# 123456jack/decision-making-and-path-planning

Measured on AMD Instinct MI355X. Metric: planning ticks/sec (batched scenes), 512x512 grid, higher is better.
Workload: dtype f64; 1 GPU; BASELINE configs[1]: 1024 scenes/GPU, 512x512 grid, 64 static obstacles; scenes_per_gpu=1024, global_scenes=1024, grid=512, obstacles=64, parallelism=scene-sharded x1, RCCL scatter/gather outside the timed region, algorithmic_bytes_per_tick=276644

## Files before the change

### decision-making-and-path-planning_amd/__init__.py

```python
import ctypes as C
import os

import numpy as np

_HERE = os.path.dirname(os.path.abspath(__file__))
LIB_PATH = os.path.join(_HERE, "libdmpp.so")

PATH_POINTS, OUT_POINTS, LANESUM, MAX_REFPATH, MAX_LATTICE = 200, 100, 8, 512, 17
GEN_LANE_PTS, GEN_REF_PTS = 320, 128

G_FOUND, G_NO_PATH, G_LIMIT, G_OVERFLOW, G_GOAL_BLOCKED, G_PATH_TRUNC, G_INTERNAL, G_COST_RANGE = range(8)
G_STATUS_COUNT = 8
K_NAMES = ["k_effective_obstacles", "k_decision", "k_planning", "k_search", "k_score"]
(BUF_SCENE_IN, BUF_LANE_POOL, BUF_REF_POOL, BUF_OBS_POOL, BUF_MOT_POOL, BUF_STATE, BUF_PLAN_OUT, BUF_GRID_OUT,
 BUF_GRID, BUF_PATH, BUF_ORDER, BUF_LANE_ATTR) = range(12)


def _dt(fields):
    return np.dtype(fields, align=True)


f8, i4, u4, f4, u8, u2 = np.float64, np.int32, np.uint32, np.float32, np.uint64, np.uint16
GlobalPoint2D = _dt([("x", f8), ("y", f8)])
GlobalPoint3D = _dt([("x", f8), ("y", f8), ("dir", f8)])
AimPoint = _dt([("Aim_point", GlobalPoint3D), ("Aim_id", i4), ("_pad", i4)])
ObPoint = _dt([("x", f8), ("y", f8), ("type", i4), ("radius", f4)])
ObMotion = _dt([("vx", f8), ("vy", f8)])
LaneView = _dt([("cur_off", i4), ("cur_n", i4), ("left_off", i4), ("left_n", i4), ("right_off", i4), ("right_n", i4),
                ("lane_sum", i4), ("lanechg_attribute", i4), ("lane_width", f8)])
LocationOut = _dt([("globalpoint", GlobalPoint3D), ("velocity", f8), ("pos", i4), ("road_num", i4), ("lane_num", i4),
                   ("last_roadnum", i4), ("next_roadnum", i4), ("last_lanenum", i4), ("next_lanenum", i4),
                   ("path_num", i4), ("id", i4, (LANESUM,))])
DecisionOutPod = _dt([("velocity_expect", f8), ("behavior", i4), ("target_roadnum", i4), ("target_lanenum", i4),
                   ("light", i4), ("behavior_to_dlg", i4), ("refpath_n", i4)])
Obs_To_Veh = _dt([("dis_lat", f8), ("dis_lng", f8)])
Path_Obs = _dt([("Ob_Pose", Obs_To_Veh), ("Ob_Attr", ObPoint), ("Obs_flag", i4), ("Ob_Pathid", i4)])
PlanningOut = _dt([("brakedis", f8), ("brake_speed", f8), ("desacc", f8), ("desspd", f8), ("desstr", f8), ("radius", f8),
                   ("cnt", i4), ("APA", i4), ("desaccVd", i4), ("desstrVd", i4), ("light", i4), ("road_type", i4),
# ... 728 lines not shown
```

### decision-making-and-path-planning_amd/csrc/dmpp_hip.hip

```cpp
#include <hip/hip_runtime.h>
#include <cstddef>
#include <cstdio>
#include <cstring>
#include <cmath>
#include <string>
#include <cstdlib>
#include <vector>
#include <new>
#include <algorithm>
#include "../../include/dmpp_planner.h"
#include "kernels_r.hpp"
#include "kernels_a.hpp"
#include "kernels_rt.hpp"
#include "kernels_ep.hpp"
#include "kernels_es.hpp"
#include "kernels_g.hpp"
#include "kernels_sc.hpp"
#include "kernels_f.hpp"
#include "kernels_t.hpp"
#include "kernels_op.hpp"
#include "search_budget.hpp"

namespace {

// ... 150 lines not shown
    DevBuf<int32_t> d_perm[kBuf], d_cost[kBuf];
    DevBuf<uint2> d_ospill[kBuf]; int spill_cap = 0; DevBuf<int32_t> d_retry[kBuf];
    hipStream_t stream_m[kBuf] = {};
    size_t grid_cells = 0;
    int bucket_cap0 = 0, max_path0 = 0;
    int search_kind = 0; int search_meta_bytes = 0; int lds_budget = 0, lds_budget_max = 0; bool lds_budget_fixed = false, search_force_gbm = false, budget_from_need = false;
    int gbm_lds = 0; int search_slots = 512; size_t search_static_lds = 0;
    DevBuf<int32_t> d_ovf[kBuf], d_need[kObs]; HostPin<int32_t> h_need;
    int need_seen = 0;
    DevBuf<int> d_gridbad;
    int gcap = 1, tick_group = 0;
    int grp_ticks = 0, grp_G = 1, grp_n = 0, grp_p_prev = 0; bool grp_piped = false;
    int grp_set[kGroupMax] = {}, grp_gs[kGroupMax] = {}; const SceneIn* grp_in = nullptr;
    int ring = 0, gring = 0;
    int item_off = 0;
    int need_set = 0;

    hipStream_t stream_r = nullptr; SyncPoint fork, join;
    SyncPoint searched[kBuf], scored[kObs], raster;
    bool front_unjoined = false;
    int parity = 0;
    bool last_piped = false;
    int obs_set = 0;
    int n_cus = 256;
    int pipeline_min = 256;
    bool r_on_main = false;
    DevBuf<char> d_scratch;
    bool streaming = false;
    InputSet in_sets[kIn]; int in_cur = 0, in_staged = -1;
    DevBuf<PlanOut> d_plan_ring[kPlan]; int plan_cur = 0;
    hipStream_t stream_up = nullptr, stream_dp = nullptr, stream_dg = nullptr;
    SyncPoint fetched_plan[kPlan], fetched_grid[kGout];
    SyncPoint done_p[kDone], done_g[kDone]; long long done_tick[kDone];
    HostPin<int32_t> h_bad;
    long long tick_seq = 0;
    TickRec rec_last = { -1, 0, nullptr, nullptr };
    std::vector<TickRec> inflight; std::vector<hipEvent_t> sync_events;
    std::vector<PendingFetch> fetches;
    RolloutState rollout;
    ScoreState score;
    FleetState fleet;
    RouteState route;
    TrafficState traffic;
    FollowState follow;
    EpisodeState episode;
    SpawnState spawn;
// ... 316 lines not shown

}

extern "C" {

const char* pp_last_error(void) { return g_err.c_str(); }

int pp_create(const PlannerConfig* cfg, int device, const PlannerCaps* caps, pp_handle* out)
{
    if (!out || !caps) return fail(PP_ERR_ARG, "null argument");
    *out = nullptr;
    int r = check_cfg(cfg); if (r) return r;
    if (caps->max_scenes <= 0) return fail(PP_ERR_ARG, "max_scenes must be positive");
    int ndev = 0;
    hipError_t e = hipGetDeviceCount(&ndev);
    if (e != hipSuccess || ndev <= 0) return fail(PP_ERR_HIP, std::string("no HIP device: ") + hipGetErrorString(e));
    if (device < 0 || device >= ndev) return fail(PP_ERR_ARG, "device index out of range");
    HIP_TRY(hipSetDevice(device));
    pp_planner* h = new (std::nothrow) pp_planner();
    if (!h) return fail(PP_ERR_HIP, "out of host memory");
    h->cfg = *cfg; h->caps = *caps; h->device = device;
    if (const char* e = std::getenv("DMPP_PIPELINE_MIN")) h->pipeline_min = std::atoi(e);
    if (const char* e = std::getenv("DMPP_TICK_GROUP")) h->tick_group = std::atoi(e);
    if (cfg->grid_stage) {
        const size_t cells = (size_t)cfg->grid_w * cfg->grid_h;
        const size_t item_bytes = cells * sizeof(uint16_t) + 3 * (cells / 32) * sizeof(uint32_t) + (size_t)std::max(caps->order_cap, 0) * sizeof(int32_t) +
                                  (cfg->bucket_cap > DMPP_OPEN_CAP ? (size_t)cfg->bucket_cap * sizeof(uint2) : 0) + 4 * sizeof(int32_t);
        h->gcap = group_cap(caps->max_scenes, h->pipeline_min, h->tick_group, item_bytes);
    }
    auto bail = [&](int code) { pp_destroy(h); return code; };
    int prio_least = 0, prio_greatest = 0;
    (void)hipDeviceGetStreamPriorityRange(&prio_least, &prio_greatest);
    const int prio_normal = (prio_least + prio_greatest) / 2;
    if (hipStreamCreateWithPriority(&h->stream, hipStreamNonBlocking, prio_normal) != hipSuccess) return bail(fail(PP_ERR_HIP, "hipStreamCreate failed"));
    h->stream_m[0] = h->stream;
    for (int q = 1; q < kBuf; q++)
        if (hipStreamCreateWithPriority(&h->stream_m[q], hipStreamNonBlocking, prio_normal) != hipSuccess) return bail(fail(PP_ERR_HIP, "hipStreamCreate failed"));
    hipDeviceProp_t prop;
    if (hipGetDeviceProperties(&prop, device) == hipSuccess) h->n_cus = prop.multiProcessorCount;
    if (hipStreamCreateWithPriority(&h->stream_r, hipStreamNonBlocking, prio_greatest) != hipSuccess) return bail(fail(PP_ERR_HIP, "hipStreamCreate failed"));
    if ((r = h->fork.create()) || (r = h->join.create())) return bail(r);
    const size_t ns = (size_t)caps->max_scenes;
    if ((r = h->in_sets[0].d_in.reserve(ns))) return bail(r);
    if ((r = h->d_lane.reserve((size_t)caps->max_lane_pts_total))) return bail(r);
    if ((r = h->d_attr.reserve((size_t)caps->max_lane_pts_total + 1))) return bail(r);
    if ((r = h->d_ref.reserve((size_t)caps->max_ref_pts_total))) return bail(r);
// ... 394 lines not shown
    const int gs = c.grid_stage ? h->gring * kGroupMax + slot : h->gout_set;
    if (h->streaming) {
        int r = pump_fetches(h, -1, (h->plan_cur + 1) % kPlan, c.grid_stage ? gs : -1); if (r) return r;
        r = prune_inflight(h); if (r) return r;
        h->plan_cur = (h->plan_cur + 1) % kPlan; h->d_plan = h->d_plan_ring[h->plan_cur];
        if (!adopted) h->h_bad[(h->tick_seq + 1) % kDone] = 0;
    }
    const TickStreams T = tick_streams(h, piped, c.grid_stage != 0, h->parity);
    hipStream_t sf = T.front, sr = T.dp;
    PP_TRY(h->scored[po].wait(sf));
    if (sf == h->stream && h->front_unjoined) PP_TRY(h->join.wait(sf));
    h->front_unjoined = false;
    if (h->r_on_main && sf != h->stream) {
        PP_TRY(h->fork.record(h->stream)); PP_TRY(h->fork.wait(sf));
    }
    h->r_on_main = sr == h->stream;
    const SyncPoint& up = h->in_sets[h->in_cur].up;
    const bool behind_upload = adopted && up.recorded();
    if (behind_upload) PP_TRY(up.wait_unless_done(sf));
    if (h->streaming) PP_TRY(h->fetched_plan[h->plan_cur].wait_unless_done(sr));
    if (h->score.ego.done()) h->score.ego.forget();
    else if (!behind_upload) PP_TRY(h->score.ego.wait(sf));
    ObPoint* obs_now = h->d_obs_now[po];
    {
        Timed t(h, PP_K_OBSTACLES, sf);
        hipLaunchKernelGGL(dmpp::k_effective_obstacles, dim3(n), dim3(dmpp::kBlock), 0, sf, c, n, h->d_in, h->d_state,
                           h->d_obs, h->have_motion ? h->d_mot : nullptr, obs_now);
    }
    if (sr != sf) { PP_TRY(h->fork.record(sf)); PP_TRY(h->fork.wait(sr)); }
    if (c.grid_stage && sf != T.search) PP_TRY(h->raster.record(sf));
    if (c.decision_stage) {
        Timed t(h, PP_K_DECISION, sr);
        hipLaunchKernelGGL(dmpp::k_decision, dim3(n), dim3(dmpp::kBlock), sizeof(dmpp::DecShared), sr, c, n, h->d_in, h->d_lane,
                           h->d_attr, h->d_ref, obs_now, h->d_state, h->d_plan, h->d_dec_ref);
    }
    {
        Timed t(h, PP_K_PLANNING, sr);
        hipLaunchKernelGGL(dmpp::k_planning, dim3(n), dim3(dmpp::kBlock), sizeof(dmpp::PlanShared), sr, c, n, h->d_in, h->d_lane,
                           h->d_ref, h->d_dec_ref, obs_now, h->d_state, h->d_plan);
    }
    if (sr != h->stream) { PP_TRY(h->join.record(sr)); h->front_unjoined = piped; }
    h->obs_set = po;
    if (c.grid_stage) {
        h->grp_set[slot] = po; h->grp_gs[slot] = gs; h->grp_in = h->d_in;
        h->grp_ticks = slot + 1;
        h->gout_set = gs; h->path_set = po;
        h->score.grp_scored = h->score.on;
        if (slot + 1 == G) { int r = flush_group(h); if (r) return r; }
    }
    h->last_piped = piped;
    h->tick_seq++;
    if (h->streaming) {
        TickRec rec = { h->tick_seq, h->in_cur, get_sync_event(h), c.grid_stage ? get_sync_event(h) : nullptr };
        if (!rec.ev_front || (c.grid_stage && !rec.ev_tail)) return fail(PP_ERR_HIP, "event creation failed");
        HIP_TRY(hipEventRecord(rec.ev_front, sr));
        if (rec.ev_tail) HIP_TRY(hipEventRecord(rec.ev_tail, T.score));
        h->inflight.push_back(rec); h->rec_last = rec;
        if (h->score.on) {
// ... 1119 lines not shown
    if (!h) return fail(PP_ERR_ARG, "null handle");
    int r = drain_events(h); if (r) return r;
    for (int k = 0; k < PP_K_COUNT; k++) { h->k_ms[k] = 0; h->k_launches[k] = 0; }
    return PP_OK;
}
void* pp_device_ptr(pp_handle h, int which, size_t* bytes)
{
    if (!h) return nullptr;
    if (flush_group(h)) return nullptr;
    const size_t ns = (size_t)h->caps.max_scenes;
    void* p = nullptr; size_t b = 0;
    switch (which) {
    case PP_BUF_SCENE_IN: p = h->d_in; b = ns * sizeof(SceneIn); break;
    case PP_BUF_LANE_POOL: p = h->d_lane; b = (size_t)h->caps.max_lane_pts_total * sizeof(GlobalPoint3D); break;
    case PP_BUF_REF_POOL: p = h->d_ref; b = (size_t)h->caps.max_ref_pts_total * sizeof(GlobalPoint2D); break;
    case PP_BUF_OBS_POOL: p = h->d_obs; b = (size_t)h->caps.max_obs_total * sizeof(ObPoint); break;
    case PP_BUF_MOT_POOL: p = h->d_mot; b = (size_t)h->caps.max_obs_total * sizeof(ObMotion); break;
    case PP_BUF_STATE: p = h->d_state; b = ns * sizeof(SceneState); break;
    case PP_BUF_PLAN_OUT: p = h->d_plan; b = ns * sizeof(PlanOut); break;
    case PP_BUF_GRID_OUT: p = h->d_gout[h->gout_set]; b = ns * sizeof(GridOut); break;
    case PP_BUF_GRID: p = nullptr; b = 0; break;
    case PP_BUF_PATH: p = h->d_path[h->path_set]; b = ns * (size_t)h->max_path0 * 4; break;
    case PP_BUF_LANE_ATTR: p = h->d_attr; b = (size_t)h->caps.max_lane_pts_total; break;
    case PP_BUF_ORDER: p = h->d_order[h->parity] ? h->d_order[h->parity] + (size_t)h->item_off * h->caps.order_cap : nullptr; b = ns * (size_t)h->caps.order_cap * 4; break;
    default: break;
    }
    if (bytes) *bytes = b;
    return p;
}
int pp_tick_group_size(int n_scenes, int search_slots, int gcap, int forced) { return group_size(n_scenes, search_slots, gcap, forced); }
int pp_tick_group_cap(int max_scenes, int pipeline_min, int forced, size_t item_bytes) { return group_cap(max_scenes, pipeline_min, forced, item_bytes); }
int pp_tick_group_const(int which)
{
    switch (which) {
    case 0: return kGroupMax;
    case 1: return kBuf;
    case 2: return kRing;
    case 3: return kObs;
    case 4: return kGoutRing;
    case 5: return kGout;
    default: return -1;
    }
}
int pp_search_budget(int static_lds, int meta_bytes, int gbm_lds, int lds_budget_max, int n_cus, int n_scenes, int group, int n_obs_total,
                     int need, int budget, int from_need, int mode, int32_t* budget_out, int32_t* from_need_out, int32_t* slots_out)
{
// ... 29 lines not shown
```

### decision-making-and-path-planning_amd/csrc/kernels_r.hpp

```cpp
#pragma once
#include "dev_geom.hpp"

#ifndef DMPP_FRONT_PRIO
#define DMPP_FRONT_PRIO 3
#endif
namespace dmpp {

constexpr int kBlock = 256;

#ifdef DMPP_DEBUG_SEARCH
#define FRONT_MARK(slot) { if (threadIdx.x == 0) dbg_stamp[slot] = (double)(clock64() - dbg_t0); }
#else
#define FRONT_MARK(slot)
#endif
constexpr int kMaxObsLds = 512;

__global__ void __launch_bounds__(kBlock)
k_effective_obstacles(PlannerConfig c, int n_scenes, const SceneIn* __restrict__ in, const SceneState* __restrict__ st,
                      const ObPoint* __restrict__ obs, const ObMotion* __restrict__ mot, ObPoint* __restrict__ now)
{
    const int s = blockIdx.x;
    if (s >= n_scenes) return;
    __builtin_amdgcn_s_setprio(3);
    const int off = in[s].obs_off, m = in[s].obs_n;
    const double t = c.dyn_dt * (double)st[s].tick;
    for (int j = threadIdx.x; j < m; j += kBlock) {
        ObPoint o = obs[off + j];
        if (c.dynamic_obstacles && mot) {
            ObMotion v = mot[off + j];
            o.x = o.x + v.vx * t;
            o.y = o.y + v.vy * t;
        }
        now[off + j] = o;
    }
}

__device__ inline int d_UpdatePlanJudge(const PlannerConfig& c, int last_behavior, int behavior, int pos,
                                        double path_lat_dis, double path_dir_err, double remain_dis, int& cause)
{
    cause = 0;
    if (last_behavior != behavior) { cause = 1; return 1; }
    if (fabs(path_lat_dis) > 0.2) { cause = 2; return 1; }
    if (fabs(path_dir_err) > 45) { cause = 3; return 1; }
    if ((pos == 0) && remain_dis < c.ROAD_REMAIN_DISTANCE) { cause = 4; return 1; }
    else if (pos != 0 && remain_dis < c.INTER_REMAIN_DISTANCE) { cause = 4; return 1; }
    return 0;
}
__device__ inline void d_SpeedPlanning(int pos, int ob_flag, double lon, float faraim, double velocity_expect,
                                       double& brakespeed, int& acc_flag, double& des_acc)
{
    if (pos == 0 || pos == 1 || pos == 2) {
        if (ob_flag) {
            if (lon - 4 > 9) { brakespeed = 3 + (lon - 9) / (faraim - 9) * (velocity_expect - 3); acc_flag = 0; des_acc = 0; }
            else if (lon - 4 > 5) { brakespeed = 3; acc_flag = 0; des_acc = 0; }
            else { brakespeed = 0; acc_flag = 1; des_acc = -3; }
        } else { brakespeed = velocity_expect; acc_flag = 0; des_acc = 0; }
    }
}
__device__ inline double d_CalculateRadius(const GlobalPoint2D* last, int near_id, int front_id)
{
    const int nid = clampi(near_id, 0, 199), f2 = clampi(front_id, 0, 199);
    const unsigned mnum = (unsigned)round((double)((nid + f2) / 2));
    const GlobalPoint2D a = last[nid], mm = last[mnum], f = last[f2];
    double dis1 = sqrt((a.x - mm.x) * (a.x - mm.x) + (a.y - mm.y) * (a.y - mm.y));
    double dis2 = sqrt((mm.x - f.x) * (mm.x - f.x) + (mm.y - f.y) * (mm.y - f.y));
    double dis3 = sqrt((a.x - f.x) * (a.x - f.x) + (a.y - f.y) * (a.y - f.y));
    double dis = dis1 * dis1 + dis2 * dis2 - dis3 * dis3;
    double cosA = dis / (2 * dis1 * dis2);
    double sinA = sqrt(1 - cosA * cosA);
    return (sinA < 0.001) ? 1000 : 0.5 * dis3 / sinA;
}

__device__ inline int block_aim_walk(const double* base, int stride, int i0, int iend, double faraim,
                                     double* seg, int* sh_found, double* sh_sum)
{
    const int tid = threadIdx.x;
    if (i0 < 0) i0 = 0;
    if (tid == 0) { *sh_found = -1; *sh_sum = 0; }
    __syncthreads();
    for (int c0 = i0; c0 < iend; c0 += kBlock) {
        const int i = c0 + tid;
        if (i < iend) {
            double dx = base[(size_t)(i + 1) * stride] - base[(size_t)i * stride];
            double dy = base[(size_t)(i + 1) * stride + 1] - base[(size_t)i * stride + 1];
            seg[tid] = sqrt(dx * dx + dy * dy);
        }
        __syncthreads();
        if (tid == 0) {
            double sum = *sh_sum;
            const int k = serial_walk(seg, iend - c0 < kBlock ? iend - c0 : kBlock, faraim, sum);
            if (k >= 0) *sh_found = c0 + k;
            *sh_sum = sum;
        }
        __syncthreads();
        if (*sh_found >= 0) break;
    }
    return *sh_found;
}

struct DecShared {
    union {
        struct {
            GlobalPoint2D F[DMPP_FRONT_POINTS], R[DMPP_REAR_POINTS], LF[DMPP_FRONT_POINTS], LR[DMPP_REAR_POINTS],
                          RF[DMPP_FRONT_POINTS], RR[DMPP_REAR_POINTS];
            GlobalPoint2D tmp[2][DMPP_FRONT_POINTS];
            double s0[DMPP_FRONT_POINTS], s1[DMPP_FRONT_POINTS];
            double seg[kBlock]; unsigned char sa[kBlock];
        } road;
        struct {
            GlobalPoint2D ref[DMPP_MAX_REFPATH];
            double s0[DMPP_MAX_REFPATH];
        } junc;
    } u;
    double part_d2[kBlock]; int part_bi[kBlock + 2];
    SoResult around[6];
    double sweep_lng[2 * DMPP_MAX_SWEEP];
    int n[6];
    int n_ref, do_sweep, n_cand;
    int rem_go, rem_flags;
    int rem_w[2][kBlock / 64]; double rem_s[2][kBlock / 64];
// ... 227 lines not shown
                            if (r) Cur.lanechg_status = 1;
                            run_left_timer(r, 2000);
                            if (LF > F + 10 && LR > 10 && left_t > 2000) { frontobs = 0; go(2, LaneNum_Cur - 1); } else keep_ns();
                        } else if (right_ok) {
                            const bool r = Cur.light_status != 2; Cur.light_status = 2;
                            run_left_timer(r, 2000);
                            if (RF > F + 10) {
                                if (RR > 10 && left_t > 2000) { frontobs = 0; go(3, 1); }
                                else keep_ns();
                            }
                        } else keep();
                    }
                } else keep();
            } else { frontobs = 0; Cur.behavior_to_dlg = 8; keep(); }
        }
    } else if (Cur.lanechg_status == 1) {
        Cur.behavior_to_dlg = 9;
        if (Cur.target_lanenum == LaneNum_Cur) Cur.lanechg_status = 0;
        Cur.behavior = st.d_his_behavior; Cur.target_lanenum = st.d_his_target_lanenum; Cur.light_status = st.d_his_light_status;
    }
    st.leftlight_time = left_t; st.rightlight_time = right_t; st.frontobs_time = frontobs;
}

__global__ void __launch_bounds__(kBlock)
k_decision(PlannerConfig c, int n_scenes, const SceneIn* __restrict__ in, const GlobalPoint3D* __restrict__ lane_pool,
           const uint8_t* __restrict__ attr_pool, const GlobalPoint2D* __restrict__ ref_pool, const ObPoint* __restrict__ obs_now,
           SceneState* __restrict__ state, PlanOut* __restrict__ plan, GlobalPoint2D* __restrict__ dec_ref)
{
    extern __shared__ __align__(16) unsigned char smem_raw[];
    DecShared& sh = *reinterpret_cast<DecShared*>(smem_raw);
    const int scene = blockIdx.x;
    if (scene >= n_scenes) return;
    __builtin_amdgcn_s_setprio(DMPP_FRONT_PRIO);
#ifdef DMPP_DEBUG_SEARCH
    const long long dbg_t0 = clock64();
    double* dbg_stamp = reinterpret_cast<double*>(dec_ref + (size_t)blockIdx.x * DMPP_MAX_REFPATH + 480);
#endif
    const int tid = threadIdx.x, wave = tid >> 6, lane = tid & 63;
    const SceneIn& si = in[scene];
    SceneState& st = state[scene];
    PlanOut& po = plan[scene];
    const LocationOut& loc = si.loc;
    const int m = si.obs_n;
    const ObPoint* obs = obs_now + si.obs_off;
    FRONT_MARK(0)
    const double hv = 0.5 * c.Vehicle_Width;
    GlobalPoint2D* out_ref = dec_ref + (size_t)scene * DMPP_MAX_REFPATH;
    const int pos = loc.pos;

    if (pos == 0) {
        const int LaneNum_Cur = loc.lane_num, LaneSum = si.lanes.lane_sum, LaneChg = si.lanes.lanechg_attribute;
        const int Id_Cur = loc.id[clampi(LaneNum_Cur - 1, 0, DMPP_LANESUM - 1)];
        const double W = si.lanes.lane_width;
        const GlobalPoint3D* cur = lane_pool + si.lanes.cur_off;
        int nF = dev_load_front(c, cur, si.lanes.cur_n, Id_Cur, sh.u.road.F);
        int nR = dev_load_rear(c, cur, si.lanes.cur_n, Id_Cur, sh.u.road.R);
        int nLF = 0, nLR = 0, nRF = 0, nRR = 0;
        int synth_left = 0, synth_right = 0;
        if (LaneChg == 1 || LaneChg == 3) {
            if (LaneNum_Cur > 1) {
                int Id_L = loc.id[clampi(LaneNum_Cur - 2, 0, DMPP_LANESUM - 1)], Sum_L = si.lanes.left_n;
                if (Id_L > 0 && Id_L < Sum_L) {
                    const GlobalPoint3D* left = lane_pool + si.lanes.left_off;
                    nLF = dev_load_front(c, left, Sum_L, Id_L, sh.u.road.LF);
                    nLR = dev_load_rear(c, left, Sum_L, Id_L, sh.u.road.LR);
                }
// ... 10 lines not shown
            } else synth_right = 1;
        }
        __syncthreads();
        if (synth_left) {
            for (int i = tid; i < nF; i += kBlock) sh.u.road.LF[i] = offset_point(c, sh.u.road.F, nF, i, -1 * W);
            for (int i = tid; i < nR; i += kBlock) sh.u.road.LR[i] = offset_point(c, sh.u.road.R, nR, i, -1 * W);
            nLF = nF; nLR = nR;
        }
        if (synth_right) {
            for (int i = tid; i < nF; i += kBlock) sh.u.road.RF[i] = offset_point(c, sh.u.road.F, nF, i, W);
            for (int i = tid; i < nR; i += kBlock) sh.u.road.RR[i] = offset_point(c, sh.u.road.R, nR, i, W);
            nRF = nF; nRR = nR;
        }
        __syncthreads();
        FRONT_MARK(1)
        const GlobalPoint2D* P[6] = { sh.u.road.F, sh.u.road.R, sh.u.road.LF, sh.u.road.LR, sh.u.road.RF, sh.u.road.RR };
        const int N[6] = { nF, nR, nLF, nLR, nRF, nRR };
        const double LO[6] = { -hv, -hv, -hv, -hv, -0.5 * W, -0.5 * W };
        const double HI[6] = { hv, hv, 0.5 * W, 0.5 * W, hv, hv };
        {
            const int team = wave >> 1;
            for (int rd = 0; rd < 3; rd++) {
                const int t = 2 * rd + team;
                const SoResult r = team_search_obstacle<2>(c, P[t], N[t], team == 0 ? sh.u.road.s0 : sh.u.road.s1, obs, m, LO[t], HI[t], true, sh.part_d2, sh.part_bi);
                if ((tid & 127) == 0) { sh.around[t] = r; sh.n[t] = N[t]; }
            }
        }
        __syncthreads();
        if (tid < 6) store_path_obs(&po.around[tid], sh.around[tid], obs, sh.n[tid] != 0);
        FRONT_MARK(2)
#ifdef DMPP_DEBUG_SEARCH
        if (tid < 6) dbg_stamp[6 + tid] = (double)sh.around[tid].adds;
#endif
        const double F_lng = (nF != 0) ? sh.around[0].dis_lng : 0.0;
        const double lim = (W - c.Vehicle_Width) / 0.6;
        int n_cand = 0;
        for (int i = 0; i < DMPP_MAX_SWEEP; i++) if ((double)i < lim) n_cand = i + 1;
        const int do_sweep = (LaneChg == 0) && (F_lng < 15) && (st.obsavoid_time + 1 > 2);
        if (do_sweep) {
            const int team = wave >> 1;
            for (int t0 = 0; t0 < 2 * n_cand; t0 += 2) {
                const int t = t0 + team;
                const bool act = t < 2 * n_cand;
                const int side = act ? t / n_cand : 0, i = act ? t - side * n_cand : 0;
                const double off = (side == 0 ? -0.3 : 0.3) * (double)i;
                if (act) for (int k = tid & 127; k < nF; k += 128) sh.u.road.tmp[team][k] = offset_point(c, sh.u.road.F, nF, k, off);
// ... 267 lines not shown
    DecisionOutPod dec;
    const GlobalPoint2D* refpath;
    if (c.decision_stage) { dec = po.dec; refpath = dec_ref + (size_t)scene * DMPP_MAX_REFPATH; }
    else {
        dec = si.dec;
        if (dec.refpath_n > si.ref_n) dec.refpath_n = si.ref_n;
        if (dec.refpath_n > DMPP_MAX_REFPATH) dec.refpath_n = DMPP_MAX_REFPATH;
        refpath = ref_pool + si.ref_off;
    }
    const GlobalPoint3D ego = loc.globalpoint;

    float faraim = 0, nearaim = 0;
    switch (pos) {
    case 0:
        faraim = (float)((loc.velocity / 3.6) * 5 + 4);
        if (faraim > c.ROAD_FARAIM_MAX) faraim = (float)c.ROAD_FARAIM_MAX;
        else if (faraim < c.ROAD_FARAIM_MIN) faraim = (float)c.ROAD_FARAIM_MIN;
        nearaim = faraim; break;
    case 1: faraim = (float)c.PRE_INTER_FARAIM; nearaim = faraim; break;
    case 2: faraim = (float)c.INTER_FARAIM; nearaim = faraim; break;
    default: break;
    }

    if (tid == 0) sh.aim_far = st.aimpoint_far;
    AimPoint aim_near_new = st.aimpoint_near;
    bool near_follows_far = false;
    {
        const int LaneNum_Cur = loc.lane_num, LaneSum = si.lanes.lane_sum;
        const int curpoint_id = loc.id[clampi(LaneNum_Cur - 1, 0, DMPP_LANESUM - 1)];
        const int curpoint_sum = si.lanes.cur_n;
        int leftpoint_id = 0, leftpoint_sum = 0, rightpoint_id = 0, rightpoint_sum = 0;
        if (LaneNum_Cur > 1) { leftpoint_id = loc.id[clampi(LaneNum_Cur - 2, 0, DMPP_LANESUM - 1)]; leftpoint_sum = si.lanes.left_n; }
        if (LaneNum_Cur < LaneSum) { rightpoint_id = loc.id[clampi(LaneNum_Cur, 0, DMPP_LANESUM - 1)]; rightpoint_sum = si.lanes.right_n; }
        const bool plan_div = !(fabs(faraim - nearaim) < 1);
        const GlobalPoint3D* cur = lane_pool + si.lanes.cur_off;
        const GlobalPoint3D* left = lane_pool + si.lanes.left_off;
        const GlobalPoint3D* right = lane_pool + si.lanes.right_off;
        __syncthreads();
        if (pos == 0) {
            if (dec.target_lanenum == loc.lane_num) {
                if (dec.behavior == 1 && !plan_div) {
                    int iend = curpoint_sum - 1;
                    int f = block_aim_walk(&cur[0].x, 3, curpoint_id, iend, (double)faraim, sh.dist, &sh.sh_found, &sh.sh_sum);
                    if (tid == 0) {
                        if (f >= 0) { sh.aim_far.Aim_point = cur[f]; sh.aim_far.Aim_id = f; }
                        else if (max(curpoint_id, 0) < iend) { sh.aim_far.Aim_point = cur[curpoint_sum - 1]; sh.aim_far.Aim_id = curpoint_sum - 1; }
                    }
                    near_follows_far = true;
                }
            } else if (dec.behavior == 2) {
                if (!plan_div) {
                    int iend = leftpoint_sum - 1;
                    int f = block_aim_walk(&left[0].x, 3, leftpoint_id, iend, (double)faraim, sh.dist, &sh.sh_found, &sh.sh_sum);
                    if (tid == 0) {
                        if (f >= 0) { sh.aim_far.Aim_point = left[f]; sh.aim_far.Aim_id = f; }
                        else if (max(leftpoint_id, 0) < iend) {
                            int q = clampi(leftpoint_sum - 2, 0, curpoint_sum > 0 ? curpoint_sum - 1 : 0);
                            sh.aim_far.Aim_point = cur[q]; sh.aim_far.Aim_id = leftpoint_sum - 1;
                        }
                    }
                }
            } else if (dec.behavior == 3) {
                if (!plan_div) {
                    int iend = min(leftpoint_sum - 1, rightpoint_sum - 1);
                    int i0 = rightpoint_id;
                    int f = (i0 >= 0) ? block_aim_walk(&right[0].x, 3, i0, iend, (double)faraim, sh.dist, &sh.sh_found, &sh.sh_sum) : -1;
                    if (tid == 0) {
                        if (f >= 0) { sh.aim_far.Aim_point = right[f]; sh.aim_far.Aim_id = f; }
                        else if (i0 >= 0 && i0 < iend) { sh.aim_far.Aim_point = right[rightpoint_sum - 1]; sh.aim_far.Aim_id = rightpoint_sum - 1; }
                    }
                }
            }
        } else if (pos == 1 || pos == 2) {
            const int n = dec.refpath_n;
            if (n >= 3) {
                int f = block_aim_walk(&refpath[0].x, 2, 0, n - 1, (double)faraim, sh.dist, &sh.sh_found, &sh.sh_sum);
                if (tid == 0) {
                    if (f >= 0) {
                        sh.aim_far.Aim_point.x = refpath[f].x; sh.aim_far.Aim_point.y = refpath[f].y;
                        if (n < 4 || f < n - 4) sh.aim_far.Aim_point.dir = GetRoadAngle(c, refpath[f], refpath[min(f + 2, n - 1)]);
                        else sh.aim_far.Aim_point.dir = GetRoadAngle(c, refpath[f - 2 < 0 ? 0 : f - 2], refpath[f]);
                        sh.aim_far.Aim_id = f;
                    } else {
                        sh.aim_far.Aim_point.x = refpath[n - 1].x; sh.aim_far.Aim_point.y = refpath[n - 1].y;
                        sh.aim_far.Aim_point.dir = GetRoadAngle(c, refpath[n - 3], refpath[n - 1]);
                        sh.aim_far.Aim_id = n - 1;
                    }
                }
            }
            near_follows_far = true;
        }
    }
    __syncthreads();
    const AimPoint aim_far = sh.aim_far;
    if (near_follows_far) aim_near_new = aim_far;

    FRONT_MARK(0)
    const int count = st.count;
    if (count == 0) {
        Bezier bz = bezier_setup(c, ego, aim_far.Aim_point);
        if (tid < DMPP_PATH_POINTS) sh.last[tid] = bezier_point(bz, tid, DMPP_PATH_POINTS);
    } else {
        if (tid < DMPP_PATH_POINTS) sh.last[tid] = st.last_Bpoints[tid];
    }
    __syncthreads();

    FRONT_MARK(1)
    if (tid < DMPP_PATH_POINTS) {
        double dx = ego.x - sh.last[tid].x, dy = ego.y - sh.last[tid].y;
        sh.dist[tid] = sqrt(dx * dx + dy * dy);
        if (tid < DMPP_PATH_POINTS - 1) {
            double sx = sh.last[tid + 1].x - sh.last[tid].x, sy = sh.last[tid + 1].y - sh.last[tid].y;
            sh.seg[tid] = sqrt(sx * sx + sy * sy);
        }
    }
    __syncthreads();
    if (wave == 0) {
        double mind = 9999; int mid = -1;
        for (int k = 0; k < 4; k++) { const int i = lane + 64 * k; if (i < DMPP_PATH_POINTS && sh.dist[i] < mind) { mind = sh.dist[i]; mid = i; } }
        wave_first_min(mind, mid);
        if (mid < 0) mid = clampi(st.path_near_id, 0, DMPP_PATH_POINTS - 1);
        const int fid = mid + 8;
      if (lane == 0) {
        const double remain = serial_sum(sh.seg, min(fid, DMPP_PATH_POINTS - 1), DMPP_PATH_POINTS - 1, 0.0);
        const int index = (mid == 199) ? mid - 1 : mid;
        const GlobalPoint2D pt = sh.last[index], pt_next = sh.last[index + 1], vp = { ego.x, ego.y };
        const double lat = GetLatDis(c, vp, pt, pt_next);
        const double pt_dir = GetRoadAngle(c, pt, pt_next);
        const double dir_err = GetAngleErr(pt_dir, ego.dir);
        int cause = 0;
        int afresh = d_UpdatePlanJudge(c, st.his_behavior, dec.behavior, pos, lat, dir_err, remain, cause);
        if (c.force_replan && !afresh) { afresh = 1; cause = 5; }
        st.path_lat_dis = lat; st.path_dir_err = dir_err; st.remain_dis = remain;
        st.path_near_id = mid; st.path_front_near_id = fid;
        st.afresh_planning = afresh; st.afresh_cause = cause;
        st.faraim_dis = faraim; st.nearaim_dis = nearaim;
        st.aimpoint_far = aim_far; st.aimpoint_near = aim_near_new;
        sh.afresh = afresh; sh.near_id = mid;
        int na = aim_far.Aim_id; if (na > 200) na = 200; if (na > dec.refpath_n) na = dec.refpath_n; if (na < 0) na = 0;
        sh.na = na;
        po.result.radius = d_CalculateRadius(sh.last, mid, fid);
      }
    }
    __syncthreads();

    FRONT_MARK(2)
    const int afresh = sh.afresh;
    if (afresh) {
        if (pos == 0) {
            Bezier bz = bezier_setup(c, ego, aim_far.Aim_point);
            if (tid < DMPP_PATH_POINTS) sh.road[tid] = bezier_point(bz, tid, DMPP_PATH_POINTS);
        } else if (pos == 1 || pos == 2) {
            const int na = sh.na;
            if (wave == 0) wave_cumlen(refpath, na, sh.s, lane);
            __syncthreads();
            if (tid < DMPP_PATH_POINTS) sh.road[tid] = mean_point(c, refpath, sh.s, na, tid, DMPP_PATH_POINTS);
        } else {
            if (tid < DMPP_PATH_POINTS) { sh.road[tid].x = 0; sh.road[tid].y = 0; }
        }
    } else {
        if (tid < DMPP_PATH_POINTS) sh.road[tid] = sh.last[tid];
    }
    __syncthreads();

    FRONT_MARK(3)
    const int near_id = clampi(sh.near_id, 0, 200);
    {
// ... 53 lines not shown
```

### include/dmpp_planner.h

```cpp
#ifndef DMPP_PLANNER_H
#define DMPP_PLANNER_H

#include "dmpp_types.h"
#include <stddef.h>

#ifdef __cplusplus
extern "C" {
#endif

#define PP_OK            0
#define PP_ERR_ARG      -1
#define PP_ERR_HIP      -2
#define PP_ERR_CAPACITY -3
#define PP_ERR_STATE    -4

#define PP_GEN_LANE_PTS 320
#define PP_GEN_REF_PTS  128

typedef struct pp_planner* pp_handle;

typedef struct PlannerCaps {
    int32_t max_scenes;
    int32_t max_obs_total;
    int32_t max_lane_pts_total;
    int32_t max_ref_pts_total;
    int32_t order_cap;
    int32_t _pad;
} PlannerCaps;

enum { PP_K_OBSTACLES = 0, PP_K_DECISION, PP_K_PLANNING, PP_K_SEARCH, PP_K_SCORE, PP_K_COUNT };
enum { PP_BUF_SCENE_IN = 0, PP_BUF_LANE_POOL, PP_BUF_REF_POOL, PP_BUF_OBS_POOL, PP_BUF_MOT_POOL, PP_BUF_STATE,
       PP_BUF_PLAN_OUT, PP_BUF_GRID_OUT, PP_BUF_GRID, PP_BUF_PATH, PP_BUF_ORDER, PP_BUF_LANE_ATTR, PP_BUF_COUNT };

const char* pp_last_error(void);

void pp_default_config(PlannerConfig* cfg, int grid_w, int grid_h);
void pp_init_state(SceneState* st, int lane_num);
int  pp_gen_scenes(const PlannerConfig* cfg, int first_scene, int n_scenes, int n_obs, int junction_every,
                   SceneIn* in, GlobalPoint3D* lane_pool, uint8_t* lane_attr_pool, GlobalPoint2D* ref_pool,
                   ObPoint* obs_pool, ObMotion* mot_pool, SceneState* state);

int  pp_create(const PlannerConfig* cfg, int device, const PlannerCaps* caps, pp_handle* out);
int  pp_destroy(pp_handle h);
int  pp_set_config(pp_handle h, const PlannerConfig* cfg);

int  pp_set_scenes(pp_handle h, int n_scenes, const SceneIn* in,
                   const GlobalPoint3D* lane_pool, const uint8_t* lane_attr_pool, int n_lane_pts,
                   const GlobalPoint2D* ref_pool, int n_ref_pts,
                   const ObPoint* obs_pool, const ObMotion* mot_pool, int n_obs_total);
int  pp_set_state(pp_handle h, const SceneState* state, int n_scenes);
int  pp_set_map(pp_handle h, const MapDesc* map);
int  pp_set_egos(pp_handle h, int n_scenes, const SceneIn* in,
                 const ObPoint* obs_pool, const ObMotion* mot_pool, int n_obs_total);
int  pp_get_scene_in(pp_handle h, SceneIn* out, int n_scenes);

// ... 115 lines not shown
```

Baseline: 5.541 million ticks/s.

## Fuse obstacle snapshot into decision kernel and overlap aim walk with path lengths

When decision and front run on the same stream and streaming is off, the effective-obstacle computation is folded into the start of k_decision, which removes one kernel launch and a global round trip per tick. The raster sync record moves after the decision kernel in the fused path. The aim-point walk is split into length and accumulate phases so that, for count>0, its first chunk overlaps with the local path-length and nearest-point work, cutting barriers. Obstacle searches with zero path points are also skipped. The cost is more code paths and a decision kernel that now writes obs_now, with a change in when search waits on the raster sync.

```diff
diff --git a/decision-making-and-path-planning_amd/__init__.py b/decision-making-and-path-planning_amd/__init__.py
--- a/decision-making-and-path-planning_amd/__init__.py
+++ b/decision-making-and-path-planning_amd/__init__.py
@@ -13,7 +13,7 @@
 G_STATUS_COUNT = 8
 K_NAMES = ["k_effective_obstacles", "k_decision", "k_planning", "k_search", "k_score"]
 (BUF_SCENE_IN, BUF_LANE_POOL, BUF_REF_POOL, BUF_OBS_POOL, BUF_MOT_POOL, BUF_STATE, BUF_PLAN_OUT, BUF_GRID_OUT,
- BUF_GRID, BUF_PATH, BUF_ORDER, BUF_LANE_ATTR) = range(12)
+ BUF_GRID, BUF_PATH, BUF_ORDER, BUF_LANE_ATTR, BUF_OBS_NOW) = range(13)
 
 
 def _dt(fields):
diff --git a/decision-making-and-path-planning_amd/csrc/dmpp_hip.hip b/decision-making-and-path-planning_amd/csrc/dmpp_hip.hip
--- a/decision-making-and-path-planning_amd/csrc/dmpp_hip.hip
+++ b/decision-making-and-path-planning_amd/csrc/dmpp_hip.hip
@@ -196,6 +196,7 @@
     int parity = 0;
     bool last_piped = false;
     int obs_set = 0;
+    bool front_snapshot = true;
     int n_cus = 256;
     int pipeline_min = 256;
     bool r_on_main = false;
@@ -558,6 +559,7 @@
     h->cfg = *cfg; h->caps = *caps; h->device = device;
     if (const char* e = std::getenv("DMPP_PIPELINE_MIN")) h->pipeline_min = std::atoi(e);
     if (const char* e = std::getenv("DMPP_TICK_GROUP")) h->tick_group = std::atoi(e);
+    if (const char* e = std::getenv("DMPP_FRONT_SNAPSHOT")) h->front_snapshot = std::atoi(e) != 0;
     if (cfg->grid_stage) {
         const size_t cells = (size_t)cfg->grid_w * cfg->grid_h;
         const size_t item_bytes = cells * sizeof(uint16_t) + 3 * (cells / 32) * sizeof(uint32_t) + (size_t)std::max(caps->order_cap, 0) * sizeof(int32_t) +
@@ -998,18 +1000,25 @@
     if (h->score.ego.done()) h->score.ego.forget();
     else if (!behind_upload) PP_TRY(h->score.ego.wait(sf));
     ObPoint* obs_now = h->d_obs_now[po];
-    {
+    const bool snap_fused = h->front_snapshot && c.decision_stage && sf == sr && !h->streaming;
+    const ObMotion* mot = h->have_motion ? h->d_mot : nullptr;
+    if (!snap_fused) {
         Timed t(h, PP_K_OBSTACLES, sf);
-        hipLaunchKernelGGL(dmpp::k_effective_obstacles, dim3(n), dim3(dmpp::kBlock), 0, sf, c, n, h->d_in, h->d_state,
-                           h->d_obs, h->have_motion ? h->d_mot : nullptr, obs_now);
+        hipLaunchKernelGGL(dmpp::k_effective_obstacles, dim3(n), dim3(dmpp::kBlock), 0, sf, c, n, h->d_in, h->d_state, h->d_obs, mot, obs_now);
     }
     if (sr != sf) { PP_TRY(h->fork.record(sf)); PP_TRY(h->fork.wait(sr)); }
-    if (c.grid_stage && sf != T.search) PP_TRY(h->raster.record(sf));
+    const bool search_waits = c.grid_stage && sf != T.search;
+    if (search_waits && !snap_fused) PP_TRY(h->raster.record(sf));
     if (c.decision_stage) {
         Timed t(h, PP_K_DECISION, sr);
-        hipLaunchKernelGGL(dmpp::k_decision, dim3(n), dim3(dmpp::kBlock), sizeof(dmpp::DecShared), sr, c, n, h->d_in, h->d_lane,
-                           h->d_attr, h->d_ref, obs_now, h->d_state, h->d_plan, h->d_dec_ref);
-    }
+        if (snap_fused)
+            hipLaunchKernelGGL(dmpp::k_decision<true>, dim3(n), dim3(dmpp::kBlock), sizeof(dmpp::DecShared), sr, c, n, h->d_in, h->d_lane,
+                               h->d_attr, h->d_ref, h->d_obs, mot, obs_now, h->d_state, h->d_plan, h->d_dec_ref);
+        else
+            hipLaunchKernelGGL(dmpp::k_decision<false>, dim3(n), dim3(dmpp::kBlock), sizeof(dmpp::DecShared), sr, c, n, h->d_in, h->d_lane,
+                               h->d_attr, h->d_ref, h->d_obs, mot, obs_now, h->d_state, h->d_plan, h->d_dec_ref);
+    }
+    if (search_waits && snap_fused) PP_TRY(h->raster.record(sf));
     {
         Timed t(h, PP_K_PLANNING, sr);
         hipLaunchKernelGGL(dmpp::k_planning, dim3(n), dim3(dmpp::kBlock), sizeof(dmpp::PlanShared), sr, c, n, h->d_in, h->d_lane,
@@ -2175,6 +2184,7 @@
     case PP_BUF_GRID: p = nullptr; b = 0; break;
     case PP_BUF_PATH: p = h->d_path[h->path_set]; b = ns * (size_t)h->max_path0 * 4; break;
     case PP_BUF_LANE_ATTR: p = h->d_attr; b = (size_t)h->caps.max_lane_pts_total; break;
+    case PP_BUF_OBS_NOW: p = h->d_obs_now[h->obs_set]; b = (size_t)h->caps.max_obs_total * sizeof(ObPoint); break;
     case PP_BUF_ORDER: p = h->d_order[h->parity] ? h->d_order[h->parity] + (size_t)h->item_off * h->caps.order_cap : nullptr; b = ns * (size_t)h->caps.order_cap * 4; break;
     default: break;
     }
diff --git a/decision-making-and-path-planning_amd/csrc/kernels_r.hpp b/decision-making-and-path-planning_amd/csrc/kernels_r.hpp
--- a/decision-making-and-path-planning_amd/csrc/kernels_r.hpp
+++ b/decision-making-and-path-planning_amd/csrc/kernels_r.hpp
@@ -15,6 +15,17 @@
 #endif
 constexpr int kMaxObsLds = 512;
 
+__device__ inline ObPoint effective_obstacle(const PlannerConfig& c, const ObPoint* __restrict__ obs, const ObMotion* __restrict__ mot, int i, double t)
+{
+    ObPoint o = obs[i];
+    if (c.dynamic_obstacles && mot) {
+        ObMotion v = mot[i];
+        o.x = o.x + v.vx * t;
+        o.y = o.y + v.vy * t;
+    }
+    return o;
+}
+
 __global__ void __launch_bounds__(kBlock)
 k_effective_obstacles(PlannerConfig c, int n_scenes, const SceneIn* __restrict__ in, const SceneState* __restrict__ st,
                       const ObPoint* __restrict__ obs, const ObMotion* __restrict__ mot, ObPoint* __restrict__ now)
@@ -24,15 +35,7 @@
     __builtin_amdgcn_s_setprio(3);
     const int off = in[s].obs_off, m = in[s].obs_n;
     const double t = c.dyn_dt * (double)st[s].tick;
-    for (int j = threadIdx.x; j < m; j += kBlock) {
-        ObPoint o = obs[off + j];
-        if (c.dynamic_obstacles && mot) {
-            ObMotion v = mot[off + j];
-            o.x = o.x + v.vx * t;
-            o.y = o.y + v.vy * t;
-        }
-        now[off + j] = o;
-    }
+    for (int j = threadIdx.x; j < m; j += kBlock) now[off + j] = effective_obstacle(c, obs, mot, off + j, t);
 }
 
 __device__ inline int d_UpdatePlanJudge(const PlannerConfig& c, int last_behavior, int behavior, int pos,
@@ -71,31 +74,32 @@
     return (sinA < 0.001) ? 1000 : 0.5 * dis3 / sinA;
 }
 
-__device__ inline int block_aim_walk(const double* base, int stride, int i0, int iend, double faraim,
-                                     double* seg, int* sh_found, double* sh_sum)
-{
-    const int tid = threadIdx.x;
-    if (i0 < 0) i0 = 0;
-    if (tid == 0) { *sh_found = -1; *sh_sum = 0; }
-    __syncthreads();
-    for (int c0 = i0; c0 < iend; c0 += kBlock) {
-        const int i = c0 + tid;
-        if (i < iend) {
-            double dx = base[(size_t)(i + 1) * stride] - base[(size_t)i * stride];
-            double dy = base[(size_t)(i + 1) * stride + 1] - base[(size_t)i * stride + 1];
-            seg[tid] = sqrt(dx * dx + dy * dy);
-        }
-        __syncthreads();
-        if (tid == 0) {
-            double sum = *sh_sum;
-            const int k = serial_walk(seg, iend - c0 < kBlock ? iend - c0 : kBlock, faraim, sum);
-            if (k >= 0) *sh_found = c0 + k;
-            *sh_sum = sum;
-        }
+__device__ inline void aim_walk_lengths(const double* base, int stride, int c0, int iend, double* seg)
+{
+    const int i = c0 + threadIdx.x;
+    if (i < iend) {
+        double dx = base[(size_t)(i + 1) * stride] - base[(size_t)i * stride];
+        double dy = base[(size_t)(i + 1) * stride + 1] - base[(size_t)i * stride + 1];
+        seg[threadIdx.x] = sqrt(dx * dx + dy * dy);
+    }
+}
+__device__ inline void aim_walk_add(const double* seg, int c0, int iend, double faraim, int* sh_found, double* sh_sum)
+{
+    double sum = *sh_sum;
+    const int k = serial_walk(seg, iend - c0 < kBlock ? iend - c0 : kBlock, faraim, sum);
+    if (k >= 0) *sh_found = c0 + k;
+    *sh_sum = sum;
+}
+__device__ inline void block_aim_walk(const double* base, int stride, int c0, int iend, double faraim,
+                                      double* seg, int* sh_found, double* sh_sum)
+{
+    for (; c0 < iend; c0 += kBlock) {
+        aim_walk_lengths(base, stride, c0, iend, seg);
+        __syncthreads();
+        if (threadIdx.x == 0) aim_walk_add(seg, c0, iend, faraim, sh_found, sh_sum);
         __syncthreads();
         if (*sh_found >= 0) break;
     }
-    return *sh_found;
 }
 
 struct DecShared {
@@ -369,9 +373,13 @@
     st.leftlight_time = left_t; st.rightlight_time = right_t; st.frontobs_time = frontobs;
 }
 
+template <bool SNAP> struct SnapshotPtr { typedef const ObPoint* __restrict__ type; };
+template <> struct SnapshotPtr<true> { typedef ObPoint* type; };
+template <bool SNAP>
 __global__ void __launch_bounds__(kBlock)
 k_decision(PlannerConfig c, int n_scenes, const SceneIn* __restrict__ in, const GlobalPoint3D* __restrict__ lane_pool,
-           const uint8_t* __restrict__ attr_pool, const GlobalPoint2D* __restrict__ ref_pool, const ObPoint* __restrict__ obs_now,
+           const uint8_t* __restrict__ attr_pool, const GlobalPoint2D* __restrict__ ref_pool,
+           const ObPoint* __restrict__ obs_pool, const ObMotion* __restrict__ mot_pool, typename SnapshotPtr<SNAP>::type obs_now,
            SceneState* __restrict__ state, PlanOut* __restrict__ plan, GlobalPoint2D* __restrict__ dec_ref)
 {
     extern __shared__ __align__(16) unsigned char smem_raw[];
@@ -389,6 +397,12 @@
     PlanOut& po = plan[scene];
     const LocationOut& loc = si.loc;
     const int m = si.obs_n;
+    if constexpr (SNAP) {
+        const double t = c.dyn_dt * (double)st.tick;
+        for (int j = tid; j < m; j += kBlock) obs_now[si.obs_off + j] = effective_obstacle(c, obs_pool, mot_pool, si.obs_off + j, t);
+        __builtin_amdgcn_s_waitcnt(0x0F70);
+        __syncthreads();
+    }
     const ObPoint* obs = obs_now + si.obs_off;
     FRONT_MARK(0)
     const double hv = 0.5 * c.Vehicle_Width;
@@ -445,6 +459,16 @@
             const int team = wave >> 1;
             for (int rd = 0; rd < 3; rd++) {
                 const int t = 2 * rd + team;
+                if (N[2 * rd] == 0 && N[2 * rd + 1] == 0) {
+                    if ((tid & 127) == 0) {
+                        SoResult z; z.flag = 0; z.path_id = 0; z.ob_index = -1; z.dis_lat = c.NO_OBSTACLE_DIS; z.dis_lng = c.NO_OBSTACLE_DIS;
+#ifdef DMPP_DEBUG_SEARCH
+                        z.adds = 0;
+#endif
+                        sh.around[t] = z; sh.n[t] = 0;
+                    }
+                    continue;
+                }
                 const SoResult r = team_search_obstacle<2>(c, P[t], N[t], team == 0 ? sh.u.road.s0 : sh.u.road.s1, obs, m, LO[t], HI[t], true, sh.part_d2, sh.part_bi);
                 if ((tid & 127) == 0) { sh.around[t] = r; sh.n[t] = N[t]; }
             }
@@ -758,107 +782,117 @@
     default: break;
     }
 
-    if (tid == 0) sh.aim_far = st.aimpoint_far;
-    AimPoint aim_near_new = st.aimpoint_near;
+    const int LaneNum_Cur = loc.lane_num, LaneSum = si.lanes.lane_sum;
+    const int curpoint_id = loc.id[clampi(LaneNum_Cur - 1, 0, DMPP_LANESUM - 1)];
+    const int curpoint_sum = si.lanes.cur_n;
+    int leftpoint_id = 0, leftpoint_sum = 0, rightpoint_id = 0, rightpoint_sum = 0;
+    if (LaneNum_Cur > 1) { leftpoint_id = loc.id[clampi(LaneNum_Cur - 2, 0, DMPP_LANESUM - 1)]; leftpoint_sum = si.lanes.left_n; }
+    if (LaneNum_Cur < LaneSum) { rightpoint_id = loc.id[clampi(LaneNum_Cur, 0, DMPP_LANESUM - 1)]; rightpoint_sum = si.lanes.right_n; }
+    const bool plan_div = !(fabs(faraim - nearaim) < 1);
+    const GlobalPoint3D* cur = lane_pool + si.lanes.cur_off;
+    const GlobalPoint3D* left = lane_pool + si.lanes.left_off;
+    const GlobalPoint3D* right = lane_pool + si.lanes.right_off;
+    int kind = 0, w_i0 = 0, w_iend = 0, w_stride = 3;
+    const double* w_base = nullptr;
     bool near_follows_far = false;
-    {
-        const int LaneNum_Cur = loc.lane_num, LaneSum = si.lanes.lane_sum;
-        const int curpoint_id = loc.id[clampi(LaneNum_Cur - 1, 0, DMPP_LANESUM - 1)];
-        const int curpoint_sum = si.lanes.cur_n;
-        int leftpoint_id = 0, leftpoint_sum = 0, rightpoint_id = 0, rightpoint_sum = 0;
-        if (LaneNum_Cur > 1) { leftpoint_id = loc.id[clampi(LaneNum_Cur - 2, 0, DMPP_LANESUM - 1)]; leftpoint_sum = si.lanes.left_n; }
-        if (LaneNum_Cur < LaneSum) { rightpoint_id = loc.id[clampi(LaneNum_Cur, 0, DMPP_LANESUM - 1)]; rightpoint_sum = si.lanes.right_n; }
-        const bool plan_div = !(fabs(faraim - nearaim) < 1);
-        const GlobalPoint3D* cur = lane_pool + si.lanes.cur_off;
-        const GlobalPoint3D* left = lane_pool + si.lanes.left_off;
-        const GlobalPoint3D* right = lane_pool + si.lanes.right_off;
-        __syncthreads();
-        if (pos == 0) {
-            if (dec.target_lanenum == loc.lane_num) {
-                if (dec.behavior == 1 && !plan_div) {
-                    int iend = curpoint_sum - 1;
-                    int f = block_aim_walk(&cur[0].x, 3, curpoint_id, iend, (double)faraim, sh.dist, &sh.sh_found, &sh.sh_sum);
-                    if (tid == 0) {
-                        if (f >= 0) { sh.aim_far.Aim_point = cur[f]; sh.aim_far.Aim_id = f; }
-                        else if (max(curpoint_id, 0) < iend) { sh.aim_far.Aim_point = cur[curpoint_sum - 1]; sh.aim_far.Aim_id = curpoint_sum - 1; }
-                    }
-                    near_follows_far = true;
-                }
-            } else if (dec.behavior == 2) {
-                if (!plan_div) {
-                    int iend = leftpoint_sum - 1;
-                    int f = block_aim_walk(&left[0].x, 3, leftpoint_id, iend, (double)faraim, sh.dist, &sh.sh_found, &sh.sh_sum);
-                    if (tid == 0) {
-                        if (f >= 0) { sh.aim_far.Aim_point = left[f]; sh.aim_far.Aim_id = f; }
-                        else if (max(leftpoint_id, 0) < iend) {
-                            int q = clampi(leftpoint_sum - 2, 0, curpoint_sum > 0 ? curpoint_sum - 1 : 0);
-                            sh.aim_far.Aim_point = cur[q]; sh.aim_far.Aim_id = leftpoint_sum - 1;
-                        }
-                    }
-                }
-            } else if (dec.behavior == 3) {
-                if (!plan_div) {
-                    int iend = min(leftpoint_sum - 1, rightpoint_sum - 1);
-                    int i0 = rightpoint_id;
-                    int f = (i0 >= 0) ? block_aim_walk(&right[0].x, 3, i0, iend, (double)faraim, sh.dist, &sh.sh_found, &sh.sh_sum) : -1;
-                    if (tid == 0) {
-                        if (f >= 0) { sh.aim_far.Aim_point = right[f]; sh.aim_far.Aim_id = f; }
-                        else if (i0 >= 0 && i0 < iend) { sh.aim_far.Aim_point = right[rightpoint_sum - 1]; sh.aim_far.Aim_id = rightpoint_sum - 1; }
-                    }
-                }
+    if (pos == 0) {
+        if (dec.target_lanenum == loc.lane_num) {
+            if (dec.behavior == 1 && !plan_div) {
+                kind = 1; w_base = &cur[0].x; w_i0 = curpoint_id; w_iend = curpoint_sum - 1;
+                near_follows_far = true;
             }
-        } else if (pos == 1 || pos == 2) {
+        } else if (dec.behavior == 2) {
+            if (!plan_div) { kind = 2; w_base = &left[0].x; w_i0 = leftpoint_id; w_iend = leftpoint_sum - 1; }
+        } else if (dec.behavior == 3) {
+            if (!plan_div) { kind = 3; w_base = &right[0].x; w_i0 = rightpoint_id; w_iend = min(leftpoint_sum - 1, rightpoint_sum - 1); }
+        }
+    } else if (pos == 1 || pos == 2) {
+        if (dec.refpath_n >= 3) { kind = 4; w_base = &refpath[0].x; w_stride = 2; w_i0 = 0; w_iend = dec.refpath_n - 1; }
+        near_follows_far = true;
+    }
+    const int w_first = max(w_i0, 0);
+    const bool walks = kind != 0 && !(kind == 3 && w_i0 < 0) && w_first < w_iend;
+    const double limit = (double)faraim;
+    double* const w_seg = sh.part_d2;
+    auto finish_aim = [&](int f) {
+        if (kind == 1) {
+            if (f >= 0) { sh.aim_far.Aim_point = cur[f]; sh.aim_far.Aim_id = f; }
+            else if (max(curpoint_id, 0) < w_iend) { sh.aim_far.Aim_point = cur[curpoint_sum - 1]; sh.aim_far.Aim_id = curpoint_sum - 1; }
+        } else if (kind == 2) {
+            if (f >= 0) { sh.aim_far.Aim_point = left[f]; sh.aim_far.Aim_id = f; }
+            else if (max(leftpoint_id, 0) < w_iend) {
+                int q = clampi(leftpoint_sum - 2, 0, curpoint_sum > 0 ? curpoint_sum - 1 : 0);
+                sh.aim_far.Aim_point = cur[q]; sh.aim_far.Aim_id = leftpoint_sum - 1;
+            }
+        } else if (kind == 3) {
+            if (f >= 0) { sh.aim_far.Aim_point = right[f]; sh.aim_far.Aim_id = f; }
+            else if (w_i0 >= 0 && w_i0 < w_iend) { sh.aim_far.Aim_point = right[rightpoint_sum - 1]; sh.aim_far.Aim_id = rightpoint_sum - 1; }
+        } else if (kind == 4) {
             const int n = dec.refpath_n;
-            if (n >= 3) {
-                int f = block_aim_walk(&refpath[0].x, 2, 0, n - 1, (double)faraim, sh.dist, &sh.sh_found, &sh.sh_sum);
-                if (tid == 0) {
-                    if (f >= 0) {
-                        sh.aim_far.Aim_point.x = refpath[f].x; sh.aim_far.Aim_point.y = refpath[f].y;
-                        if (n < 4 || f < n - 4) sh.aim_far.Aim_point.dir = GetRoadAngle(c, refpath[f], refpath[min(f + 2, n - 1)]);
-                        else sh.aim_far.Aim_point.dir = GetRoadAngle(c, refpath[f - 2 < 0 ? 0 : f - 2], refpath[f]);
-                        sh.aim_far.Aim_id = f;
-                    } else {
-                        sh.aim_far.Aim_point.x = refpath[n - 1].x; sh.aim_far.Aim_point.y = refpath[n - 1].y;
-                        sh.aim_far.Aim_point.dir = GetRoadAngle(c, refpath[n - 3], refpath[n - 1]);
-                        sh.aim_far.Aim_id = n - 1;
-                    }
-                }
+            if (f >= 0) {
+                sh.aim_far.Aim_point.x = refpath[f].x; sh.aim_far.Aim_point.y = refpath[f].y;
+                if (n < 4 || f < n - 4) sh.aim_far.Aim_point.dir = GetRoadAngle(c, refpath[f], refpath[min(f + 2, n - 1)]);
+                else sh.aim_far.Aim_point.dir = GetRoadAngle(c, refpath[f - 2 < 0 ? 0 : f - 2], refpath[f]);
+                sh.aim_far.Aim_id = f;
+            } else {
+                sh.aim_far.Aim_point.x = refpath[n - 1].x; sh.aim_far.Aim_point.y = refpath[n - 1].y;
+                sh.aim_far.Aim_point.dir = GetRoadAngle(c, refpath[n - 3], refpath[n - 1]);
+                sh.aim_far.Aim_id = n - 1;
             }
-            near_follows_far = true;
-        }
-    }
-    __syncthreads();
-    const AimPoint aim_far = sh.aim_far;
-    if (near_follows_far) aim_near_new = aim_far;
-
-    FRONT_MARK(0)
-    const int count = st.count;
-    if (count == 0) {
-        Bezier bz = bezier_setup(c, ego, aim_far.Aim_point);
-        if (tid < DMPP_PATH_POINTS) sh.last[tid] = bezier_point(bz, tid, DMPP_PATH_POINTS);
-    } else {
-        if (tid < DMPP_PATH_POINTS) sh.last[tid] = st.last_Bpoints[tid];
-    }
-    __syncthreads();
-
-    FRONT_MARK(1)
-    if (tid < DMPP_PATH_POINTS) {
-        double dx = ego.x - sh.last[tid].x, dy = ego.y - sh.last[tid].y;
-        sh.dist[tid] = sqrt(dx * dx + dy * dy);
-        if (tid < DMPP_PATH_POINTS - 1) {
-            double sx = sh.last[tid + 1].x - sh.last[tid].x, sy = sh.last[tid + 1].y - sh.last[tid].y;
-            sh.seg[tid] = sqrt(sx * sx + sy * sy);
-        }
-    }
-    __syncthreads();
-    if (wave == 0) {
-        double mind = 9999; int mid = -1;
+        }
+    };
+    auto local_lengths = [&]() {
+        if (tid < DMPP_PATH_POINTS) {
+            double dx = ego.x - sh.last[tid].x, dy = ego.y - sh.last[tid].y;
+            sh.dist[tid] = sqrt(dx * dx + dy * dy);
+            if (tid < DMPP_PATH_POINTS - 1) {
+                double sx = sh.last[tid + 1].x - sh.last[tid].x, sy = sh.last[tid + 1].y - sh.last[tid].y;
+                sh.seg[tid] = sqrt(sx * sx + sy * sy);
+            }
+        }
+    };
+    int mid = -1; double remain = 0;
+    auto local_nearest = [&]() {
+        double mind = 9999;
         for (int k = 0; k < 4; k++) { const int i = lane + 64 * k; if (i < DMPP_PATH_POINTS && sh.dist[i] < mind) { mind = sh.dist[i]; mid = i; } }
         wave_first_min(mind, mid);
         if (mid < 0) mid = clampi(st.path_near_id, 0, DMPP_PATH_POINTS - 1);
+        if (lane == 0) remain = serial_sum(sh.seg, min(mid + 8, DMPP_PATH_POINTS - 1), DMPP_PATH_POINTS - 1, 0.0);
+    };
+
+    const int count = st.count;
+    if (tid == 0) { sh.aim_far = st.aimpoint_far; sh.sh_found = -1; sh.sh_sum = 0; }
+    if (count == 0) {
+        __syncthreads();
+        if (walks) block_aim_walk(w_base, w_stride, w_first, w_iend, limit, w_seg, &sh.sh_found, &sh.sh_sum);
+        if (tid == 0) finish_aim(sh.sh_found);
+        __syncthreads();
+        FRONT_MARK(0)
+        Bezier bz = bezier_setup(c, ego, sh.aim_far.Aim_point);
+        if (tid < DMPP_PATH_POINTS) sh.last[tid] = bezier_point(bz, tid, DMPP_PATH_POINTS);
+        __syncthreads();
+        local_lengths();
+        __syncthreads();
+        if (wave == 0) local_nearest();
+        FRONT_MARK(1)
+    } else {
+        if (tid < DMPP_PATH_POINTS) sh.last[tid] = st.last_Bpoints[tid];
+        if (walks) aim_walk_lengths(w_base, w_stride, w_first, w_iend, w_seg);
+        __syncthreads();
+        local_lengths();
+        __syncthreads();
+        FRONT_MARK(0)
+        if (wave == 0) local_nearest();
+        else if (tid == 64 && walks) aim_walk_add(w_seg, w_first, w_iend, limit, &sh.sh_found, &sh.sh_sum);
+        __syncthreads();
+        if (walks && sh.sh_found < 0)
+            block_aim_walk(w_base, w_stride, w_first + kBlock, w_iend, limit, w_seg, &sh.sh_found, &sh.sh_sum);
+        if (tid == 0) finish_aim(sh.sh_found);
+        FRONT_MARK(1)
+    }
+    if (tid == 0) {
+        const AimPoint aim_far = sh.aim_far;
         const int fid = mid + 8;
-      if (lane == 0) {
-        const double remain = serial_sum(sh.seg, min(fid, DMPP_PATH_POINTS - 1), DMPP_PATH_POINTS - 1, 0.0);
         const int index = (mid == 199) ? mid - 1 : mid;
         const GlobalPoint2D pt = sh.last[index], pt_next = sh.last[index + 1], vp = { ego.x, ego.y };
         const double lat = GetLatDis(c, vp, pt, pt_next);
@@ -871,14 +905,15 @@
         st.path_near_id = mid; st.path_front_near_id = fid;
         st.afresh_planning = afresh; st.afresh_cause = cause;
         st.faraim_dis = faraim; st.nearaim_dis = nearaim;
-        st.aimpoint_far = aim_far; st.aimpoint_near = aim_near_new;
+        st.aimpoint_far = aim_far;
+        if (near_follows_far) st.aimpoint_near = aim_far;
         sh.afresh = afresh; sh.near_id = mid;
         int na = aim_far.Aim_id; if (na > 200) na = 200; if (na > dec.refpath_n) na = dec.refpath_n; if (na < 0) na = 0;
         sh.na = na;
         po.result.radius = d_CalculateRadius(sh.last, mid, fid);
-      }
     }
     __syncthreads();
+    const AimPoint aim_far = sh.aim_far;
 
     FRONT_MARK(2)
     const int afresh = sh.afresh;
diff --git a/include/dmpp_planner.h b/include/dmpp_planner.h
--- a/include/dmpp_planner.h
+++ b/include/dmpp_planner.h
@@ -30,7 +30,7 @@
 
 enum { PP_K_OBSTACLES = 0, PP_K_DECISION, PP_K_PLANNING, PP_K_SEARCH, PP_K_SCORE, PP_K_COUNT };
 enum { PP_BUF_SCENE_IN = 0, PP_BUF_LANE_POOL, PP_BUF_REF_POOL, PP_BUF_OBS_POOL, PP_BUF_MOT_POOL, PP_BUF_STATE,
-       PP_BUF_PLAN_OUT, PP_BUF_GRID_OUT, PP_BUF_GRID, PP_BUF_PATH, PP_BUF_ORDER, PP_BUF_LANE_ATTR, PP_BUF_COUNT };
+       PP_BUF_PLAN_OUT, PP_BUF_GRID_OUT, PP_BUF_GRID, PP_BUF_PATH, PP_BUF_ORDER, PP_BUF_LANE_ATTR, PP_BUF_OBS_NOW, PP_BUF_COUNT };
 
 const char* pp_last_error(void);
 
```

Result: faster. 5.658 million ticks/s, median of 6 (+2.1%).
